# COMBINE-lab/RapMap

Measured on AMD Instinct MI355X. Metric: Mreads/s (paired 2x100 bp; one unit = one read pair), higher is better.
Workload: dtype u8/int32/u64 (integer & byte work, no floating point)

## Files before the change

rapmap_amd/csrc/qm_device.h:

```cpp
#pragma once
#include <hip/hip_runtime.h>
#include <stddef.h>
#include <cstdlib>
#include "qm_grid.h"

#define QM_SEL_CHUNKS_B 4
#define QMK_DEFAULT_WPS 8
#define QMK_WPS_PH 6
#define QMK_WPS_NIP 8
#define QMK_WPS_PHNIP 6

namespace qm {
struct DevIndex; struct ReadBatch; struct PairBatch; struct SelBatch;
struct EqcSrc;

template <auto K, int THREADS, int FALLBACK, bool KNOB>
inline int resident_per_cu() {
  static const int nb = [] {
    int v = 0;
    if (hipOccupancyMaxActiveBlocksPerMultiprocessor(&v, K, THREADS, 0) != hipSuccess || v < 1) v = FALLBACK;
    const char* ov = KNOB ? getenv("QM_BLOCKS_PER_CU") : nullptr;
    if (ov && atoi(ov) > 0 && atoi(ov) < v) v = atoi(ov);
    return v;
  }();
  return nb;
}
}

hipError_t qmk_build_sainfo(const unsigned int* SA, long long nSA, const unsigned int* offsets, long long T, void* out, hipStream_t st);
hipError_t qmk_build_saext(const unsigned char* text, long long n, const unsigned int* SA, long long nSA, int k, const void* sainfo, void* out, hipStream_t st);
hipError_t qmk_build_saext2(const unsigned char* text, long long n, const unsigned int* SA, long long nSA, int k, const void* sainfo, void* out, hipStream_t st);
hipError_t qmk_build_sanext(const unsigned char* text, long long n, const unsigned int* SA, long long nSA, int k, unsigned int* out, hipStream_t st);
hipError_t qmk_build_slots(const void* recs, long long K, void* slots, unsigned long long cap, int k, hipStream_t st);
hipError_t qmk_build_slots_from_ph(const qm::DevIndex& ix, long long n, void* slots, unsigned long long cap, unsigned long long* d_bad, hipStream_t st);
hipError_t qmk_build_phrecs(const unsigned int* data, const unsigned char* lens, long long n, const qm::DevIndex& ix, void* out, hipStream_t st);
hipError_t qmk_build_phfilter(const void* recs, long long n, void* filter, unsigned long long mask, int k, hipStream_t st);
enum ReadLaunch {
  RL_FUSED,
  RL_CHAIN_COLLECT,
  RL_ENTRY_COLLECT,
  RL_LONG,
  RL_LONG_COLLECT
};
hipError_t qmk_map_reads(const qm::DevIndex& ix, const qm::ReadBatch& B, int ns, ReadLaunch what, int grid, int num_cu, hipStream_t st);
hipError_t qmk_launch_reads_ns2(const qm::DevIndex& ix, const qm::ReadBatch& B, bool collect, int grid, int num_cu, hipStream_t st);
hipError_t qmk_launch_reads_ns3(const qm::DevIndex& ix, const qm::ReadBatch& B, bool collect, int grid, int num_cu, hipStream_t st);
hipError_t qmk_launch_reads_ns4(const qm::DevIndex& ix, const qm::ReadBatch& B, bool collect, int grid, int num_cu, hipStream_t st);
hipError_t qmk_launch_reads_ns8(const qm::DevIndex& ix, const qm::ReadBatch& B, bool collect, int grid, int num_cu, hipStream_t st);
hipError_t qmk_launch_reads_ns32(const qm::DevIndex& ix, const qm::ReadBatch& B, bool collect, int grid, int num_cu, hipStream_t st);
hipError_t qmk_launch_lean(const qm::DevIndex& ix, const qm::ReadBatch& B, int num_cu, hipStream_t st);
hipError_t qmk_launch_lean_nq(const qm::DevIndex& ix, const qm::ReadBatch& B, int num_cu, hipStream_t st);
hipError_t qmk_launch_duo(const qm::DevIndex& ix, const qm::ReadBatch& B, int num_cu, hipStream_t st);
hipError_t qmk_h2m(const qm::DevIndex& ix, const qm::ReadBatch& B, int grid, int num_cu, hipStream_t st);
hipError_t qmk_h2m_packw(const qm::DevIndex& ix, const qm::ReadBatch& B, const long long* ids, const unsigned long long* nids, long long* todoq, int grid, int num_cu, hipStream_t st);
hipError_t qmk_h2m_pack(const qm::DevIndex& ix, const qm::ReadBatch& B, long long* todoq, int grid, int num_cu, hipStream_t st);
hipError_t qmk_sel_merge(const qm::PairBatch& P, const qm::SelBatch& A, hipStream_t st);
hipError_t qmk_collect_marked(const unsigned int* lcnt, long long nreads, unsigned int mark, long long* q, long long cap, unsigned long long* count, hipStream_t st);
hipError_t qmk_sel_slots(const qm::PairBatch& P, hipStream_t st);
hipError_t qmk_sel_plan(const qm::PairBatch& P, const qm::SelBatch& A, int num_cu, hipStream_t st);
hipError_t qmk_sel_align_finish(const qm::PairBatch& P, const qm::SelBatch& A, int num_cu, hipStream_t st);
size_t qmk_sel_gmem_rows_bytes(int num_cu);
hipError_t qmk_sel_compact(const qm::PairBatch& P, const void* tmp, const void* toff, hipStream_t st);
hipError_t qmk_pair_count(const qm::PairBatch& P, hipStream_t st);
hipError_t qmk_pair_write(const qm::PairBatch& P, hipStream_t st);
hipError_t qmk_unpack_reads(const unsigned char* packed, const long long* off, long long n, long long total_chars, unsigned char* seq,
                            const void* exc, long long n_exc, hipStream_t st);
size_t qmk_scan_temp_bytes(long long n);
hipError_t qmk_scan_counts(void* temp, size_t temp_bytes, const unsigned int* cnt, long long* offs, long long n, long long init,
                           hipStream_t st);
hipError_t qmk_scan_counts_masked(void* temp, size_t temp_bytes, const unsigned int* cnt, long long* offs, long long n, hipStream_t st);
hipError_t qmk_stage_gather(long long nreads, const unsigned int* ivcnt, const long long* ivoff, const void* iv, const long long* ivcsr, void* iv_out,
                            const unsigned int* lcnt, const long long* loff, const unsigned long long* lists, const long long* lcsr,
                            unsigned long long* words_out, hipStream_t st);

hipError_t qmk_eqc_label_queued(const qm::EqcSrc& src, long long nq, hipStream_t st);
hipError_t qmk_eqc_reset_probes(unsigned long long* q, long long n, hipStream_t st);
hipError_t qmk_eqc_sum(const unsigned long long* count, const unsigned long long* key, long long cap, unsigned long long* out, hipStream_t st);
```

rapmap_amd/csrc/qm_grid.h:

```cpp
#pragma once
#include <cstdlib>

namespace qm {

constexpr int GRID_NOMINAL_PER_CU = 8;

inline int grid_oversub() {
  static const int m = [] { const char* e = getenv("QM_GRID_OVERSUB"); return e && atoi(e) > 0 && atoi(e) <= 16 ? atoi(e) : 4; }();
  return m;
}
inline int grid_oversub_ph() {
  static const int m = [] { const char* e = getenv("QM_GRID_OVERSUB_PH"); return e && atoi(e) > 0 && atoi(e) <= 16 ? atoi(e) : (getenv("QM_GRID_OVERSUB") ? grid_oversub() : 12); }();
  return m;
}

inline int grid_clamp(long long blocks, int num_cu, int resident_per_cu, int oversub) {
  const long long cap = (long long)num_cu * resident_per_cu * oversub;
  const long long g = blocks < cap ? blocks : cap;
  return (int)(g > 0 ? g : 1);
}
inline int grid_blocks(long long work, int num_cu, int resident_per_cu, int oversub) { return grid_clamp((work + 3) / 4, num_cu, resident_per_cu, oversub); }

inline long long lean_iters(long long nreads, bool wide) { return wide ? nreads : (nreads + 1) >> 1; }
inline long long pair_iters(long long nreads) { return nreads >> 1; }

inline int map_grid(long long nreads, int num_cu, bool ph_compact) { return grid_blocks(nreads, num_cu, GRID_NOMINAL_PER_CU, ph_compact ? grid_oversub_ph() : grid_oversub()); }
inline int resident_grid(long long nreads, int num_cu) { return grid_blocks(nreads, num_cu, GRID_NOMINAL_PER_CU, 1); }

inline int sweep_grid(long long lanes, int num_cu, int resident_per_cu, int max_blocks) {
  const int g = grid_blocks((lanes + 63) / 64, num_cu > 0 ? num_cu : 1, resident_per_cu, 1);
  return max_blocks > 0 && g > max_blocks ? max_blocks : g;
}

}
```

rapmap_amd/csrc/qm_kernels_duo.hip:

```cpp
#include <hip/hip_runtime.h>
#include <cstdlib>
#include "qm_duo.inl"
#include "qm_device.h"

namespace qm {

template <bool PH, bool COV>
__global__ __launch_bounds__(256, 8) void qm_duo_kernel(DevIndex ix_, ReadBatch B_) {
  const DevIndex& ix = stage_args().ix; const ReadBatch& B = stage_args().B;
  __shared__ __attribute__((aligned(16))) DuoMem mem[4];
  const int wave = __builtin_amdgcn_readfirstlane((int)(threadIdx.x >> 6));
  duo_wave<PH, COV>(ix, B, (int)blockIdx.x * 4 + wave, (int)gridDim.x * 4, mem[wave]);
}

}

using namespace qm;

hipError_t qmk_launch_duo(const DevIndex& ix, const ReadBatch& B, int num_cu, hipStream_t st) {
  if (!B.seq2 || (B.nreads & 1)) return hipErrorInvalidValue;
  static const int knob = [] { const char* e = getenv("QM_DUO_OVERSUB"); return e && atoi(e) > 0 ? atoi(e) : 0; }();
  return duo_dispatch(ix.ph != nullptr, B.quasi_cov > 0.0, [&](auto ph, auto cov) {
    constexpr bool PH = decltype(ph)::value, COV = decltype(cov)::value;
    const int over = knob ? knob : (PH ? grid_oversub_ph() : 2 * grid_oversub());
    const int g = grid_blocks(pair_iters(B.nreads), num_cu, resident_per_cu<qm_duo_kernel<PH, COV>, 256, 8, true>(), over);
    hipLaunchKernelGGL((qm_duo_kernel<PH, COV>), dim3((unsigned)g), dim3(256), 0, st, ix, B);
    return hipGetLastError();
  });
}
```

Measured before the change: 494.5.

## Launch duo kernel as single-wave workgroups with contiguous per-wave trip runs

The pair-mapping kernel now launches one-wave workgroups (QM_WG_WAVES=1) instead of 256-thread blocks, with four times as many blocks and one wave's shared DuoMem each. A run-shift parameter groups consecutive trips into runs of up to 8 per wave, so each wave processes contiguous pairs before striding across the grid. Occupancy is re-queried per wave. The aim is to cut the workgroup-level coupling and load imbalance of 4-wave blocks and to improve locality of read accesses. A profiling summary script is also added. Risks are more dispatch overhead for small blocks and a tail imbalance from coarser runs. The duo_wave signature change lives in a file not shown.

```diff
diff --git a/profiles/wave_runs/summarize.py b/profiles/wave_runs/summarize.py
--- /dev/null
+++ b/profiles/wave_runs/summarize.py
@@ -0,0 +1,123 @@
+#!/usr/bin/env python3
+import collections
+import csv
+import glob
+import gzip
+import json
+import os
+import shutil
+import statistics as st
+import sys
+
+OUT = sys.argv[1]
+PRUNE = "--prune" in sys.argv[2:]
+PAIRS = 1e7
+
+
+def short(k):
+    return k.split("(")[0].replace("void ", "").replace("qm::", "").split("<")[0]
+
+
+def rows(pattern):
+    out = []
+    for f in sorted(glob.glob(os.path.join(OUT, pattern), recursive=True)):
+        with (gzip.open(f, "rt") if f.endswith(".gz") else open(f)) as h:
+            out += list(csv.DictReader(h))
+    return out
+
+
+def keep(name, pattern):
+    files = sorted(glob.glob(os.path.join(OUT, pattern), recursive=True))
+    if not files:
+        return
+    os.makedirs(os.path.join(OUT, "raw"), exist_ok=True)
+    with gzip.open(os.path.join(OUT, "raw", name + ".csv.gz"), "wt") as o:
+        head = False
+        for f in files:
+            with open(f) as h:
+                first = h.readline()
+                if not head:
+                    o.write(first)
+                    head = True
+                for line in h:
+                    if "qm_" in line or "qm::" in line:
+                        o.write(line)
+
+
+def bench_tables():
+    print("# bench.py lines by variant: M pairs/s (ms_per_step, map_kernel_ms), in the order they were measured")
+    for f in sorted(glob.glob(os.path.join(OUT, "*.jsonl"))):
+        v, ms, km = [], [], []
+        for line in open(f):
+            line = line.strip()
+            if not line.startswith("{"):
+                continue
+            d = json.loads(line)
+            v.append(d["value"]); ms.append(d["ms_per_step"]); km.append(d.get("config", {}).get("map_kernel_ms"))
+        if not v:
+            continue
+        name = os.path.basename(f)[:-6]
+        print("%-14s n %d  min %.1f  median %.1f  max %.1f  mean %.1f  spread %.1f M pairs/s;  ms_per_step median %.3f;  map_kernel_ms median %s"
+              % (name, len(v), min(v), st.median(v), max(v), st.mean(v), max(v) - min(v), st.median(ms),
+                 "%.3f" % st.median([k for k in km if k is not None]) if any(k is not None for k in km) else "-"))
+        print("   " + "  ".join("%.1f (%.3f, %s)" % (a, b, c) for a, b, c in zip(v, ms, km)))
+
+
+def trace_tables():
+    for v in ("parent", "branch"):
+        name = "trace_" + v
+        r = rows("raw/%s.csv.gz" % name) or rows("%s/**/*kernel_trace.csv" % name)
+        if not r:
+            continue
+        by = collections.defaultdict(list)
+        for x in r:
+            if "qm" in x["Kernel_Name"]:
+                by[short(x["Kernel_Name"])].append((int(x["Start_Timestamp"]), int(x["End_Timestamp"])))
+        print("# kernel trace, %s: python bench.py --gpus 1 --steps 10 --warmup 3 under rocprofv3 --kernel-trace --stats" % v)
+        for k in sorted(by, key=lambda k: -sum(e - s for s, e in by[k])):
+            d = [(e - s) / 1e6 for s, e in by[k]]
+            print("   %-28s dispatches %4d  mean %8.3f ms  median %8.3f ms  total %9.3f ms" % (k, len(d), st.mean(d), st.median(d), sum(d)))
+        duo, lean = sorted(by.get("qm_duo_kernel", [])), sorted(by.get("qm_lean_kernel", []))
+        if duo and lean:
+            spans = []
+            for s, e in duo:
+                over = [(ls, le) for ls, le in lean if ls < e and le > s]
+                if over:
+                    spans.append((max([e] + [le for ls, le in over]) - min([s] + [ls for ls, le in over])) / 1e6)
+            if spans:
+                print("   stage-A span (pair kernel with the lean launches that overlap it): n %d  mean %.3f ms  median %.3f ms" % (len(spans), st.mean(spans), st.median(spans)))
+
+
+def pmc_tables():
+    print("# counters per dispatch of each kernel alone over the 10 M pairs (QM_SPLIT=1; lean: QM_NO_DUO=1, pair: QM_DUO_PARTS=-1), per pair in brackets")
+    for kern, kname in (("duo", "qm_duo_kernel"), ("lean", "qm_lean_kernel")):
+        for v in ("parent", "branch"):
+            tot, n = collections.Counter(), collections.Counter()
+            for p in ("sq", "tcc"):
+                name = "pmc_%s_%s_%s" % (v, kern, p)
+                for x in rows("raw/%s.csv.gz" % name) or rows("%s/**/*counter_collection.csv" % name):
+                    if short(x["Kernel_Name"]) == kname:
+                        tot[x["Counter_Name"]] += float(x["Counter_Value"]); n[x["Counter_Name"]] += 1
+            if not tot:
+                continue
+            per = {c: tot[c] / n[c] for c in tot}
+            print("%s, %s (%d dispatches):" % (kname, v, max(n.values())))
+            for c in sorted(per):
+                print("   %-18s %16.0f  (%9.3f)" % (c, per[c], per[c] / PAIRS))
+            if per.get("SQ_BUSY_CYCLES"):
+                print("   slot fill SQ_WAVE_CYCLES x 4 / SQ_BUSY_CYCLES / 256 = %.4f" % (per["SQ_WAVE_CYCLES"] * 4 / per["SQ_BUSY_CYCLES"] / 256))
+
+
+if PRUNE:
+    for d in sorted(glob.glob(os.path.join(OUT, "trace_*")) + glob.glob(os.path.join(OUT, "pmc_*"))):
+        if os.path.isdir(d):
+            keep(os.path.basename(d), os.path.basename(d) + ("/**/*kernel_trace.csv" if "trace_" in d else "/**/*counter_collection.csv"))
+            shutil.rmtree(d)
+    for d in glob.glob(os.path.join(OUT, "dump_*")):
+        if os.path.isdir(d):
+            shutil.rmtree(d)
+for part in (bench_tables, trace_tables, pmc_tables):
+    try:
+        part()
+    except Exception as e:
+        print("# %s: %s: %s" % (part.__name__, type(e).__name__, e))
diff --git a/rapmap_amd/csrc/qm_device.h b/rapmap_amd/csrc/qm_device.h
--- a/rapmap_amd/csrc/qm_device.h
+++ b/rapmap_amd/csrc/qm_device.h
@@ -1,6 +1,7 @@
 #pragma once
 #include <hip/hip_runtime.h>
 #include <stddef.h>
+#include <cstdio>
 #include <cstdlib>
 #include "qm_grid.h"
 
@@ -24,6 +25,20 @@
     return v;
   }();
   return nb;
+}
+template <auto K, int FALLBACK>
+inline int resident_quads_per_cu(const char* name) {
+  static const int nq = [name] {
+    int v = 0;
+    const bool asked = hipOccupancyMaxActiveBlocksPerMultiprocessor(&v, K, 64 * QM_WG_WAVES, 0) == hipSuccess && v >= 1;
+    if (getenv("QM_GRID_TRACE")) fprintf(stderr, "[qm grid] %s: %d workgroups of %d wave(s) resident per CU%s\n", name, asked ? v : 0, QM_WG_WAVES, asked ? "" : " (the query failed)");
+    v = asked ? v * QM_WG_WAVES / 4 : FALLBACK;
+    if (v < 1) v = 1;
+    const char* ov = getenv("QM_BLOCKS_PER_CU");
+    if (ov && atoi(ov) > 0 && atoi(ov) < v) v = atoi(ov);
+    return v;
+  }();
+  return nq;
 }
 }
 
diff --git a/rapmap_amd/csrc/qm_grid.h b/rapmap_amd/csrc/qm_grid.h
--- a/rapmap_amd/csrc/qm_grid.h
+++ b/rapmap_amd/csrc/qm_grid.h
@@ -27,6 +27,41 @@
 inline int map_grid(long long nreads, int num_cu, bool ph_compact) { return grid_blocks(nreads, num_cu, GRID_NOMINAL_PER_CU, ph_compact ? grid_oversub_ph() : grid_oversub()); }
 inline int resident_grid(long long nreads, int num_cu) { return grid_blocks(nreads, num_cu, GRID_NOMINAL_PER_CU, 1); }
 
+#ifndef QM_WG_WAVES
+#define QM_WG_WAVES 1
+#endif
+#if defined(__HIPCC__) && !defined(QM_EMU)
+#define QM_GRID_FN __host__ __device__ inline
+#else
+#define QM_GRID_FN inline
+#endif
+constexpr int WAVE_RUN_MAX = 8;
+constexpr int WAVE_RUN_DEFAULT = 8;
+
+inline int wave_run() {
+  static const int r = [] { const char* e = getenv("QM_WAVE_RUN"); const int v = e ? atoi(e) : 0; return v == 1 || v == 2 || v == 4 || v == 8 ? v : WAVE_RUN_DEFAULT; }();
+  return r;
+}
+inline int wave_blocks(int quads, int wg_waves) { return quads * (4 / wg_waves); }
+QM_GRID_FN long long run_count(long long trips, int rs) { return (trips + (1LL << rs) - 1) >> rs; }
+inline int run_shift(long long trips, long long resident_waves, int want) {
+  int rs = 0;
+  while ((2 << rs) <= want && (2 << rs) <= WAVE_RUN_MAX && run_count(trips, rs + 1) >= resident_waves) ++rs;
+  return rs;
+}
+struct WaveGrid { int blocks, rs; };
+inline WaveGrid wave_grid(long long trips, int num_cu, int quads_per_cu, int oversub) {
+  const WaveGrid g = {wave_blocks(grid_blocks(trips, num_cu, quads_per_cu, oversub), QM_WG_WAVES), run_shift(trips, 4LL * num_cu * quads_per_cu, wave_run())};
+  return g;
+}
+QM_GRID_FN long long run_trip(long long t, int gw, int nw, int rs) { return ((((t >> rs) * nw) + gw) << rs) + (t & ((1LL << rs) - 1)); }
+QM_GRID_FN int run_ends(int it, int trips, int rs) { return (it + 1 >= trips || ((it + 1) & ((1 << rs) - 1)) == 0) ? 1 : 0; }
+QM_GRID_FN int run_ahead(int it, int trips, int nw, int rs, int ahead) {
+  const unsigned n = ((unsigned)(it >> rs) + (unsigned)ahead * (unsigned)nw) << rs;
+  return n < (unsigned)trips ? (int)n : trips;
+}
+QM_GRID_FN int run_next(int it, int trips, int nw, int rs) { return run_ends(it, trips, rs) ? run_ahead(it, trips, nw, rs, 1) : it + 1; }
+
 inline int sweep_grid(long long lanes, int num_cu, int resident_per_cu, int max_blocks) {
   const int g = grid_blocks((lanes + 63) / 64, num_cu > 0 ? num_cu : 1, resident_per_cu, 1);
   return max_blocks > 0 && g > max_blocks ? max_blocks : g;
diff --git a/rapmap_amd/csrc/qm_kernels_duo.hip b/rapmap_amd/csrc/qm_kernels_duo.hip
--- a/rapmap_amd/csrc/qm_kernels_duo.hip
+++ b/rapmap_amd/csrc/qm_kernels_duo.hip
@@ -6,11 +6,11 @@
 namespace qm {
 
 template <bool PH, bool COV>
-__global__ __launch_bounds__(256, 8) void qm_duo_kernel(DevIndex ix_, ReadBatch B_) {
+__global__ __launch_bounds__(64 * QM_WG_WAVES, 8) void qm_duo_kernel(DevIndex ix_, ReadBatch B_, int rs) {
   const DevIndex& ix = stage_args().ix; const ReadBatch& B = stage_args().B;
-  __shared__ __attribute__((aligned(16))) DuoMem mem[4];
-  const int wave = __builtin_amdgcn_readfirstlane((int)(threadIdx.x >> 6));
-  duo_wave<PH, COV>(ix, B, (int)blockIdx.x * 4 + wave, (int)gridDim.x * 4, mem[wave]);
+  __shared__ __attribute__((aligned(16))) DuoMem mem[QM_WG_WAVES];
+  const int wave = QM_WG_WAVES == 1 ? 0 : __builtin_amdgcn_readfirstlane((int)(threadIdx.x >> 6));
+  duo_wave<PH, COV>(ix, B, (int)blockIdx.x * QM_WG_WAVES + wave, (int)gridDim.x * QM_WG_WAVES, mem[wave], rs);
 }
 
 }
@@ -23,8 +23,8 @@
   return duo_dispatch(ix.ph != nullptr, B.quasi_cov > 0.0, [&](auto ph, auto cov) {
     constexpr bool PH = decltype(ph)::value, COV = decltype(cov)::value;
     const int over = knob ? knob : (PH ? grid_oversub_ph() : 2 * grid_oversub());
-    const int g = grid_blocks(pair_iters(B.nreads), num_cu, resident_per_cu<qm_duo_kernel<PH, COV>, 256, 8, true>(), over);
-    hipLaunchKernelGGL((qm_duo_kernel<PH, COV>), dim3((unsigned)g), dim3(256), 0, st, ix, B);
+    const WaveGrid g = wave_grid(pair_iters(B.nreads), num_cu, resident_quads_per_cu<qm_duo_kernel<PH, COV>, 8>("qm_duo_kernel"), over);
+    hipLaunchKernelGGL((qm_duo_kernel<PH, COV>), dim3((unsigned)g.blocks), dim3(64 * QM_WG_WAVES), 0, st, ix, B, g.rs);
     return hipGetLastError();
   });
 }
```

After: 506.6, median of 6. +2.4%, better.
